# terryye/cuda_FlashAttention

Hardware: AMD Instinct MI355X
Metric: FA2 fwd+bwd TFLOP/s at (B=4,H=16,N=8192,d=128); % MFMA peak (higher is better)
Workload: dtype bf16; 1 GPU; FA2 forward+backward bf16, (B=4,H=16,N=8192,d=128) per GPU, non-causal (BASELINE configs[2]); flops = 14 B H N^2 d; B=4, H=16, N=8192, d=128, parallelism=head-sharded replicas x1

## Files before the change

cuda_flashattention_amd/csrc/fa2_bwd_bf16.hip:

```cpp
#include <type_traits>

#include "fa2_regfile.h"
#include "fa2_launch.h"

namespace fa2 {

constexpr float kNoKeyRC = -1.0e30f;
constexpr float kNoKeyLq = 1.0e30f;

template <int D>
__global__ void __launch_bounds__(256) fa2_bwd_delta_kernel(const __bf16* __restrict__ dO,
                                                            const __bf16* __restrict__ O,
                                                            const float* __restrict__ L,
                                                            float* __restrict__ Dv, float* __restrict__ RC,
                                                            size_t rows, int nq, int q_hs, int q_row0, size_t rc_plane,
                                                            float inv_scale)
{
    const size_t r = ((size_t)blockIdx.x * 256 + threadIdx.x) >> 4;
    const int sub = threadIdx.x & 15;
    const size_t head = r / (size_t)nq, i = r % (size_t)nq;
    const size_t row = head * (size_t)q_hs + i;
    const size_t prow = row + (size_t)q_row0;
    float acc = 0.0f;
    if (r < rows) {
#pragma unroll
        for (int c = sub * 8; c < D; c += 128) {
            const bf16x8 a = *reinterpret_cast<const bf16x8*>(dO + row * D + c);
            const bf16x8 b = *reinterpret_cast<const bf16x8*>(O + row * D + c);
#pragma unroll
            for (int e = 0; e < 8; ++e) acc += (float)a[e] * (float)b[e];
        }
    }
#pragma unroll
    for (int off = 8; off >= 1; off >>= 1) acc += __shfl_xor(acc, off, 16);
    if (r < rows && sub == 0) {
        Dv[prow] = acc;
        const float l = L[row];
        RC[prow] = l == -INFINITY ? kNoKeyRC : -l * inv_scale;
        RC[rc_plane + prow] = -acc;
    }
}

constexpr int kBwdRows = 256;
constexpr int kDqWaves = 4;
constexpr int kDqKV = 64;
constexpr int kDkQ = 32;

typedef __attribute__((address_space(3))) void* lptr_t;

#include "fa2_bwd_dq_body.inc"
// ... 402 lines not shown
            constexpr int RK = A_DK + 16 * (kb * DT + dt) + 4 * g, RV = A_DV + 16 * (kb * DT + dt) + 4 * g;
            bf16x4 a, b;
            a[0] = (__bf16)(aread<RK>() * p.scale); a[1] = (__bf16)(aread<RK + 1>() * p.scale);
            a[2] = (__bf16)(aread<RK + 2>() * p.scale); a[3] = (__bf16)(aread<RK + 3>() * p.scale);
            b[0] = (__bf16)aread<RV>(); b[1] = (__bf16)aread<RV + 1>();
            b[2] = (__bf16)aread<RV + 2>(); b[3] = (__bf16)aread<RV + 3>();
            if (key < N) {
                *reinterpret_cast<bf16x4*>(dKk + 2 * (32 * dt + 8 * g + 4 * h)) = a;
                *reinterpret_cast<bf16x4*>(dVk + 2 * (32 * dt + 8 * g + 4 * h)) = b;
            }
        });
    });
}

template <int D, bool CAUSAL>
__global__ void __launch_bounds__(256, 1) __attribute__((amdgpu_num_vgpr(60))) fa2_bwd_dkdv_kernel(BwdArgs p)
{
    const int ncb = (p.Nk + kDkKeys - 1) / kDkKeys;
    int kvhead, cb;
    map_block(blockIdx.x, p.BH / p.kv_group, ncb, kvhead, cb);
    bwd_dkdv_impl<D, CAUSAL>(p, kvhead, cb);
}

template <int D, bool CAUSAL>
__global__ void __launch_bounds__(256, 1) __attribute__((amdgpu_num_vgpr(60))) fa2_bwd_dkdv_varlen_kernel(VarlenBwdArgs v)
{
    int kvhead, idx;
    map_block(blockIdx.x, v.a.BH / v.a.kv_group, v.n_key_items, kvhead, idx);
    const VarlenItem it = uniform_item(v.key_items, idx);
    bwd_dkdv_impl<D, CAUSAL>(bwd_varlen_view<D>(v.a, it), kvhead, it.block);
}

template <int D, bool CAUSAL>
static hipError_t launch_bwd_one(const BwdArgs& a, hipStream_t stream)
{
    const size_t rows = (size_t)a.BH * a.Nq;
    hipError_t e = hipSuccess;
    if (a.phases & 1) {
        hipLaunchKernelGGL((fa2_bwd_delta_kernel<D>), dim3((unsigned)((rows * 16 + 255) / 256)), dim3(256), 0,
                           stream, (const __bf16*)a.dO, (const __bf16*)a.O, a.L, a.D, a.RC, rows, a.Nq, a.q_hs, a.q_row0,
                           (size_t)a.BH * a.q_hs, 1.0f / a.scale);
        e = hipGetLastError();
        if (e != hipSuccess) return e;
    }
    const int nb = (a.Nq + kBwdRows - 1) / kBwdRows;
    constexpr int lds_dq = 3 * 2 * kDqKV * D * 2;
    constexpr int lds_dk = kDkKeys * D * 2 + 2 * (2 * 2 * kDkQ * D * 2 + 512);
    if (a.phases & 2) {
        e = launch_lds<fa2_bwd_dq_kernel<D, CAUSAL>>(dim3((unsigned)(nb * a.BH)), dim3(256), lds_dq, stream, a);
        if (e != hipSuccess) return e;
    }
    if (a.phases & 4) {
        const int ncb = (a.Nk + kDkKeys - 1) / kDkKeys;
        e = launch_lds<fa2_bwd_dkdv_kernel<D, CAUSAL>>(dim3((unsigned)(ncb * (a.BH / a.kv_group))), dim3(256), lds_dk, stream, a);
    }
    return e;
}

template <int D, bool CAUSAL>
static hipError_t launch_bwd_varlen_one(const VarlenBwdArgs& v, hipStream_t stream)
{
    const BwdArgs& a = v.a;
    const size_t rows = (size_t)a.BH * a.q_hs;
    hipLaunchKernelGGL((fa2_bwd_delta_kernel<D>), dim3((unsigned)((rows * 16 + 255) / 256)), dim3(256), 0, stream,
                       (const __bf16*)a.dO, (const __bf16*)a.O, a.L, a.D, a.RC, rows, a.q_hs, a.q_hs, 0, rows, 1.0f / a.scale);
    hipError_t e = hipGetLastError();
    if (e != hipSuccess) return e;
    constexpr int lds_dq = 3 * 2 * kDqKV * D * 2;
    constexpr int lds_dk = kDkKeys * D * 2 + 2 * (2 * 2 * kDkQ * D * 2 + 512);
    e = launch_lds<fa2_bwd_dq_varlen_kernel<D, CAUSAL>>(dim3((unsigned)(v.n_row_items * a.BH)), dim3(256), lds_dq, stream, v);
    if (e != hipSuccess) return e;
    return launch_lds<fa2_bwd_dkdv_varlen_kernel<D, CAUSAL>>(dim3((unsigned)(v.n_key_items * (a.BH / a.kv_group))), dim3(256), lds_dk,
                                                            stream, v);
}

hipError_t launch_bwd_varlen_bf16(const VarlenBwdArgs& v, hipStream_t stream)
{
    const BwdArgs& a = v.a;
    if (a.kv_group < 1 || a.BH % a.kv_group != 0 || v.n_row_items < 1 || v.n_key_items < 1 || !v.row_items || !v.key_items)
        return hipErrorInvalidValue;
    if (a.d == 128) return a.causal ? launch_bwd_varlen_one<128, true>(v, stream) : launch_bwd_varlen_one<128, false>(v, stream);
    if (a.d == 64) return a.causal ? launch_bwd_varlen_one<64, true>(v, stream) : launch_bwd_varlen_one<64, false>(v, stream);
    return hipErrorInvalidValue;
}

hipError_t launch_bwd_bf16(const BwdArgs& a, hipStream_t stream)
{
    if (a.kv_group < 1 || a.BH % a.kv_group != 0) return hipErrorInvalidValue;
    if (a.d == 128) return a.causal ? launch_bwd_one<128, true>(a, stream) : launch_bwd_one<128, false>(a, stream);
    if (a.d == 64) return a.causal ? launch_bwd_one<64, true>(a, stream) : launch_bwd_one<64, false>(a, stream);
    return hipErrorInvalidValue;
}

}
```

cuda_flashattention_amd/csrc/fa2_bwd_fused.hip:

```cpp
#include <cstdlib>
#include <cstring>
#include <type_traits>

#include "fa2_regfile.h"
#include "fa2_launch.h"

namespace fa2 {

#include "fa2_bwd_fused_body.inc"

typedef __attribute__((address_space(3))) void* fused_lptr_t;

#ifndef FA2_FUSED_DSKEY
#define FA2_FUSED_DSKEY(row) (((row) >> 1) & 7)
#endif

#ifndef FA2_FUSED_DIAG
#define FA2_FUSED_DIAG 0
#endif

constexpr int kFusedRegFile = RF512;

#define FA2_FUSED_CLOBBERS "memory", "vcc", FA2_RF512
#define FA2_FUSED_OPS_128 [r0] "v"(roff[0]), [r1] "v"(roff[1]), [r2] "v"(roff[2]), [r3] "v"(roff[3]), [r4] "v"(roff[4]), [r5] "v"(roff[5]),  \
    [r6] "v"(roff[6]), [r7] "v"(roff[7]), [t0] "v"(toff[0]), [t1] "v"(toff[1]), [t2] "v"(toff[2]), [t3] "v"(toff[3]), [t4] "v"(toff[4]),   \
    [t5] "v"(toff[5]), [t6] "v"(toff[6]), [t7] "v"(toff[7]), [rc] "v"(rcv), [c2] "s"(c2)
#define FA2_FUSED_OPS_64 [r0] "v"(roff[0]), [r1] "v"(roff[1]), [r2] "v"(roff[2]), [r3] "v"(roff[3]), [t0] "v"(toff[0]), [t1] "v"(toff[1]),    \
    [t2] "v"(toff[2]), [t3] "v"(toff[3]), [rc] "v"(rcv), [c2] "s"(c2)

struct FusedStep {
    __amdgpu_buffer_rsrc_t drs, lrs, qrs, grs, rcrs, ctl;
    uint32_t dso, lso, qso, rcso, pvo, mso;
    int need, pval;
};
#define FA2_FUSED_STEP(TEXT, DD, ...)                                                                                                 \
    asm volatile(TEXT                                                                                                                 \
                 : [err] "+s"(err)                                                                                                    \
                 : FA2_FUSED_OPS_##DD, [vm] "i"(VMW), [dqv] "v"(dqv), [drs] "s"(f.drs), [dso] "s"(f.dso), [lrs] "s"(f.lrs), [lso] "s"(f.lso), \
// ... 27 lines not shown

template <int DQT>
__device__ __forceinline__ void fused_dq_atomic(__amdgpu_buffer_rsrc_t rs, uint32_t voff, uint32_t soff)
{
    asm volatile(
        "s_add_u32 s12, %2, 4096\n\ts_add_u32 s13, %2, 8192\n\ts_add_u32 s14, %2, 12288\n\t"
        "buffer_atomic_add_f32 v%c3, %0, %1, %2 offen\n\tbuffer_atomic_add_f32 v%c4, %0, %1, %2 offen offset:512\n\t"
        "buffer_atomic_add_f32 v%c5, %0, %1, %2 offen offset:1024\n\tbuffer_atomic_add_f32 v%c6, %0, %1, %2 offen offset:1536\n\t"
        "buffer_atomic_add_f32 v%c7, %0, %1, s12 offen\n\tbuffer_atomic_add_f32 v%c8, %0, %1, s12 offen offset:512\n\t"
        "buffer_atomic_add_f32 v%c9, %0, %1, s12 offen offset:1024\n\tbuffer_atomic_add_f32 v%c10, %0, %1, s12 offen offset:1536\n\t"
        "buffer_atomic_add_f32 v%c11, %0, %1, s13 offen\n\tbuffer_atomic_add_f32 v%c12, %0, %1, s13 offen offset:512\n\t"
        "buffer_atomic_add_f32 v%c13, %0, %1, s13 offen offset:1024\n\tbuffer_atomic_add_f32 v%c14, %0, %1, s13 offen offset:1536\n\t"
        "buffer_atomic_add_f32 v%c15, %0, %1, s14 offen\n\tbuffer_atomic_add_f32 v%c16, %0, %1, s14 offen offset:512\n\t"
        "buffer_atomic_add_f32 v%c17, %0, %1, s14 offen offset:1024\n\tbuffer_atomic_add_f32 v%c18, %0, %1, s14 offen offset:1536\n\t"
        "s_nop 1"
        : : "v"(voff), "s"(rs), "s"(soff), "i"(DQT), "i"(DQT + 1), "i"(DQT + 2), "i"(DQT + 3), "i"(DQT + 4), "i"(DQT + 5), "i"(DQT + 6),
            "i"(DQT + 7), "i"(DQT + 8), "i"(DQT + 9), "i"(DQT + 10), "i"(DQT + 11), "i"(DQT + 12), "i"(DQT + 13), "i"(DQT + 14),
            "i"(DQT + 15)
        : "memory", "s12", "s13", "s14", "v255");
}

template <int VF, int KS, int S>
__device__ __forceinline__ void fused_load_vfrag(const char* v0, const char* v1)
{
#ifndef FA2_FUSED_KV_NT
#define FA2_FUSED_KV_NT ""
#define FA2_FUSED_KV_AUX 0
#endif
    asm volatile("global_load_dwordx4 v[%c2:%c3], %0, off offset:%c4" FA2_FUSED_KV_NT "\n\tglobal_load_dwordx4 v[%c5:%c6], %1, off offset:%c4" FA2_FUSED_KV_NT
                 : : "v"(v0), "v"(v1), "i"(VF + 4 * S), "i"(VF + 4 * S + 3), "i"(32 * S), "i"(VF + 4 * (KS + S)), "i"(VF + 4 * (KS + S) + 3)
                 : "memory", "v255");
}

template <int DQT>
__device__ __forceinline__ void fused_dq_zero()
{
    static_for<16>([&](auto R) { vset<kFusedRegFile, CL_TOP, DQT + decltype(R)::value>(0u); });
}

constexpr int kCtlTicket = 0, kCtlNextHead = 32 * 16, kCtlError = 32 * 17, kCtlHeadmap = 32 * 18;
constexpr int kHmPad = 16;
constexpr int kSpinLimit = FA2_FUSED_SPIN_LIMIT;

struct FusedArgs {
    BwdArgs b;
    float* dQacc;
    int* ctl;
    int npad;
    const float* rc;
    int fault;
};

#ifdef FA2_TEST_HOOKS
static int g_hook_fault = 0, g_hook_grid = 0, g_hook_last_grid = 0;
extern "C" void fa2_test_set_fused_hooks(int fault, int grid) { g_hook_fault = fault; g_hook_grid = grid; }
extern "C" int fa2_test_last_fused_grid(void) { return g_hook_last_grid; }
#define FA2_HOOK_NOTE_GRID(n) (g_hook_last_grid = (n))
#else
constexpr int g_hook_fault = 0, g_hook_grid = 0;
#define FA2_HOOK_NOTE_GRID(n) ((void)0)
#endif

__device__ __forceinline__ int fused_ctl_ints(int BH, int ncb) { return kCtlHeadmap + 16 * (BH + kHmPad) + 9 * BH * ncb; }

__device__ __forceinline__ int fused_load_sc1(const int* p)
{
    int v;
    asm volatile("global_load_dword %0, %1, off sc1\n\ts_waitcnt vmcnt(0)" : "=v"(v) : "v"(p) : "memory");
    return v;
}
__device__ __forceinline__ void fused_seen_set(int v)
{
    asm volatile("v_mov_b32 v39, %0" : : "s"(v) : "v39");
}

__device__ __forceinline__ int fused_lane_id() { return (int)__builtin_amdgcn_mbcnt_hi(~0u, __builtin_amdgcn_mbcnt_lo(~0u, 0u)); }
template <int OFF>
__device__ __forceinline__ int fused_mail_read(uint32_t lds_addr)
{
    int v;
    asm volatile("v_mov_b32 %0, %1\n\tds_read_b32 %0, %0 offset:%c2\n\ts_waitcnt lgkmcnt(0)" : "=&v"(v) : "s"(lds_addr), "i"(OFF) : "memory");
    return __builtin_amdgcn_readfirstlane(v);
}

__device__ __forceinline__ void fused_store_flag(int* p, int v)
{
    asm volatile("global_store_dword %0, %1, off" : : "v"(p), "v"(v) : "memory");
}

__device__ __forceinline__ bool fused_spin_over(int* ctl, int spins)
{
    if (spins > kSpinLimit) {
        atomicExch(ctl + kCtlError, 1);
        return true;
    }
    return (spins & 1023) == 0 && fused_load_sc1(ctl + kCtlError) != 0;
}

template <bool CHAIN, bool CAUSAL, bool RAGGED = false, bool RECT = false, int HD = 128>
__global__ void __launch_bounds__(256, 1) __attribute__((amdgpu_num_vgpr(39))) fa2_bwd_fused_kernel(FusedArgs fp)
{
    static_assert(CHAIN || !RAGGED, "the atomics form has no ragged variant");
    static_assert(!RECT || (CHAIN && !CAUSAL && !RAGGED), "rectangular blocks: chained, unmasked, aligned");
    static_assert(HD == 128 || (HD == 64 && CHAIN && !RECT), "head_dim 64: chained, square");
    extern __shared__ __attribute__((aligned(16))) char smem[];
    const BwdArgs& p = fp.b;
// ... 37 lines not shown
    for (int dt = 0; dt < DT; ++dt)
#pragma unroll
        for (int jj = 0; jj < 2; ++jj)
            toff[2 * dt + jj] = lbase + QRING + lds_off<D>(8 * jj + 4 * h + trq, 4 * dt + 2 * trcb + (trp >> 1)) + 8 * (trp & 1);
    const uint32_t rcv = lbase + QRING + 2 * TROWS * ROWB + 16 * h;
    static_for<KS>([&](auto S) {
        constexpr int sidx = decltype(S)::value;
        vset<kFusedRegFile, CL_TOP, ROFFK + sidx>(lbase + lds_off<D>(ki + 64 * wave, 2 * sidx + h));
    });
    const int ecol = W ? wave : (wave & 1), ekey0 = W ? 0 : 128 * (wave >> 1);
    static_for<2>([&](auto JJ) {
        constexpr int jj = decltype(JJ)::value;
        vset<kFusedRegFile, CL_TOP, KT + jj>(lbase + ekey0 * ROWB + lds_off<D>(8 * jj + 4 * h + trq, 4 * ecol + 2 * trcb + (trp >> 1)) + 8 * (trp & 1));
        const int row = 8 * jj + 4 * h + trq;
        vset<kFusedRegFile, CL_TOP, DSRD + jj>(lbase + DSB + (ekey0 + row) * 64 + 8 * ((4 * trcb + trp) ^ FA2_FUSED_DSKEY(row)));
    });
    static_for<4>([&](auto C) {
        constexpr int c = decltype(C)::value;
        vset<kFusedRegFile, CL_TOP, DSWR + c>(lbase + DSB + (64 * wave + ki) * 64 + 8 * (((2 * c) | h) ^ FA2_FUSED_DSKEY(ki)));
    });
    const int doff = lds_dma_off<D>(wave * RPI, lane);
    const uint32_t dqv = CHAIN ? (uint32_t)(wave * 4096 + lane * 16) : (uint32_t)(((4 * h) * D + 32 * wave + ki) * 4);
    const auto rc_rsrc = __builtin_amdgcn_make_buffer_rsrc((void*)fp.rc, 0, (int)(2 * rc_plane * 4), 0x00020000);

    int xcc = 0;
    if constexpr (CHAIN) {
        asm volatile("s_getreg_b32 %0, hwreg(HW_REG_XCC_ID, 0, 4)" : "=s"(xcc));
    }
    int* const prog_base = fp.ctl + kCtlHeadmap + 16 * (p.BH + kHmPad);
#ifndef FA2_FUSED_CAUSAL_G
#define FA2_FUSED_CAUSAL_G 2
#endif
    const int G = CAUSAL ? max(1, min(FA2_FUSED_CAUSAL_G, p.BH / 8)) : 1;
    const auto ctl_rsrc = __builtin_amdgcn_make_buffer_rsrc((void*)fp.ctl, 0, CHAIN ? fused_ctl_ints(p.BH, ncb) * 4 : 0, 0x00020000);

    auto take_ticket = [&]() {
        if (wave == 0 && fused_lane_id() == 0) {
            int hd, j = 0;
            do {
                const int u = atomicAdd(fp.ctl + kCtlTicket + 32 * xcc, 1);
                const int r = u % (G * ncb);
                const int k = (u / (G * ncb)) * G + r % G;
                j = r / G;
                hd = -2;
                if (k < p.BH + kHmPad) {
                    int* hm = fp.ctl + kCtlHeadmap + xcc * (p.BH + kHmPad) + k;
                    int v = 0, spins = 0;
                    if (j == 0) {
                        if (k > 0)
                            while ((v = fused_load_sc1(hm - 1)) == 0)
                                if (fused_spin_over(fp.ctl, ++spins)) break;
                        if (k > 0 && v == 0) {
                            v = -1;
                        } else {
                            const int g = atomicAdd(fp.ctl + kCtlNextHead, 1);
                            v = g < p.BH ? g + 1 : -1;
                        }
                        fused_store_flag(hm, v);
                    } else {
                        while ((v = fused_load_sc1(hm)) == 0)
                            if (fused_spin_over(fp.ctl, ++spins)) { v = -1; break; }
                    }
                    hd = v > 0 ? v - 1 : (r % G == 0 ? -2 : -1);
                }
            } while (hd == -1);
            mail[0] = hd;
            mail[1] = j;
            mail[2] = hd >= 0 ? fused_load_sc1(fp.ctl + kCtlError) : 0;
        }
    };
    auto issue_unit_loads = [&](int head_, int cb_) {
        const size_t slab_ = (size_t)(head_ / p.kv_group) * KHS * ROWB;
        const char* Kh_ = (const char*)p.K + slab_;
        const char* Vh_ = (const char*)p.V + slab_;
        const int kw0_ = cb_ * 256 + wave * 64;
        const int lane_u = (int)__builtin_amdgcn_mbcnt_hi(~0u, __builtin_amdgcn_mbcnt_lo(~0u, 0u));
        const int vk0 = RAGGED ? min(kw0_ + (lane_u & 31), N - 1) : kw0_ + (lane_u & 31);
        const int vk1 = RAGGED ? min(kw0_ + 32 + (lane_u & 31), N - 1) : kw0_ + 32 + (lane_u & 31);
        const char* v0 = Vh_ + (size_t)vk0 * ROWB + 16 * (lane_u >> 5);
        const char* v1 = Vh_ + (size_t)vk1 * ROWB + 16 * (lane_u >> 5);
        static_for<KS>([&](auto S) { fused_load_vfrag<VF, KS, decltype(S)::value>(v0, v1); });
        const auto k_rsrc = __builtin_amdgcn_make_buffer_rsrc((void*)Kh_, 0, N * ROWB, 0x00020000);
#pragma unroll
        for (int j = wave; j < 256 / RPI; j += 4)
            __builtin_amdgcn_raw_ptr_buffer_load_lds(k_rsrc, (fused_lptr_t)(smem + j * 1024), 16, doff, (cb_ * 256 + j * RPI) * ROWB, 0, FA2_FUSED_KV_AUX);
    };

    auto next_unit_loads = [&]() {
        if constexpr (CHAIN) {
            take_ticket();
            __syncthreads();
            const int hn = fused_mail_read<0>(mail_addr);
            if (hn >= 0) issue_unit_loads(hn, fused_mail_read<4>(mail_addr));
        }
    };
    next_unit_loads();

    for (;;) {
#ifdef FA2_FUSED_STATS
        const uint64_t s_pull = __builtin_readcyclecounter();
#endif
        int head, cb, err0 = 0;
        if constexpr (CHAIN) {
            head = fused_mail_read<0>(mail_addr);
            cb = fused_mail_read<4>(mail_addr);
            err0 = fused_mail_read<8>(mail_addr);
            if (head < 0) break;
        } else {
            map_block(blockIdx.x, p.BH, ncb, head, cb);
            issue_unit_loads(head, cb);
        }
        const size_t slab = (size_t)head * QHS * ROWB;
        const char* Qh = (const char*)p.Q + slab;
        const char* Gh = (const char*)p.dO + slab;
        const int kw0 = cb * 256 + wave * 64;
        {
            const u32x4 z = {0u, 0u, 0u, 0u};
            static_for<4 * DT>([&](auto T) { azero16<kFusedRegFile, CL_ACC, 16 * decltype(T)::value>(z); });
        }

        const auto q_rsrc = __builtin_amdgcn_make_buffer_rsrc((void*)Qh, 0, NQ * ROWB, 0x00020000);
        const auto g_rsrc = __builtin_amdgcn_make_buffer_rsrc((void*)Gh, 0, NQ * ROWB, 0x00020000);
        const int rcoff = (int)(((wave == 0 ? 0 : rc_plane) + (size_t)head * (RECT ? QHS : NP) + QR0 + (fused_lane_id() & 31)) * 4);
        auto stage = [&](int t, int buf) {
            char* b = smem + QRING + buf * BUFB;
#pragma unroll
            for (int j = wave; j < 2 * NINS; j += 4) {
                const int which = j / NINS, piece = j % NINS;
                const int soff = (t * TROWS + piece * RPI) * ROWB;
                __builtin_amdgcn_raw_ptr_buffer_load_lds(which ? g_rsrc : q_rsrc, (fused_lptr_t)(b + which * (TROWS * ROWB) + piece * 1024),
                                                         16, doff, soff, 0, 0);
            }
            if (wave < 2 && fused_lane_id() < 32)
                __builtin_amdgcn_raw_ptr_buffer_load_lds(rc_rsrc, (fused_lptr_t)(b + 2 * TROWS * ROWB + wave * 128), 4, rcoff, t * TROWS * 4, 0, 0);
        };
        const int n_u = CAUSAL ? ntiles - 8 * cb : ntiles;
        const int niter_u = CAUSAL ? ((n_u + 1 + 5) / 6) * 6 : niter;
        const bool ragged_unit = RAGGED && !CAUSAL && cb == ncb - 1;
        const int first_masked = CAUSAL ? ((n_u - 8) / 6) * 6 : (ragged_unit ? 0 : niter_u);
// ... 91 lines not shown
#endif
                fused_dq_zero<DQT>();
            }
        };
        auto six = [&](auto MASKED, auto FAST_, int t) {
            step(std::integral_constant<int, 0>{}, std::integral_constant<int, 0>{}, MASKED, FAST_, t);
            step(std::integral_constant<int, 1>{}, std::integral_constant<int, 1>{}, MASKED, FAST_, t + 1);
            step(std::integral_constant<int, 2>{}, std::integral_constant<int, 0>{}, MASKED, FAST_, t + 2);
            step(std::integral_constant<int, 0>{}, std::integral_constant<int, 1>{}, MASKED, FAST_, t + 3);
            step(std::integral_constant<int, 1>{}, std::integral_constant<int, 0>{}, MASKED, FAST_, t + 4);
            step(std::integral_constant<int, 2>{}, std::integral_constant<int, 1>{}, MASKED, FAST_, t + 5);
        };
        const int fast_end = CHAIN ? n_u - 2 : -1;
        {
            const int plain_end = first_masked;
            int t = 0;
            asm volatile("" : "+s"(t));
            if (t < plain_end) { six(std::false_type{}, std::false_type{}, t); t += 6; }
#pragma unroll 1
            for (; t + 5 <= fast_end && t < plain_end; t += 6) six(std::false_type{}, std::true_type{}, t);
#pragma unroll 1
            for (; t < plain_end; t += 6) six(std::false_type{}, std::false_type{}, t);
            if constexpr (CHAIN && (CAUSAL || RAGGED)) {
#pragma unroll 1
                for (; t < niter_u; t += 6) six(std::true_type{}, std::false_type{}, t);
            }
        }
        asm volatile("s_waitcnt vmcnt(0) lgkmcnt(0)" ::: "memory");
        if constexpr (CHAIN)
            if (err && !err0 && wave == 0 && fused_lane_id() == 0) atomicExch(fp.ctl + kCtlError, 1);
#ifdef FA2_FUSED_STATS
        const uint64_t s_loop = __builtin_readcyclecounter();
#endif
        next_unit_loads();

        mfma_acc_settle();
        const int lane_ep = (int)__builtin_amdgcn_mbcnt_hi(~0u, __builtin_amdgcn_mbcnt_lo(~0u, 0u));
        const int ki_ep = lane_ep & 31, h_ep = lane_ep >> 5;
        static_for<2>([&](auto KB) {
            constexpr int kb = decltype(KB)::value;
            const int key = kw0 + 32 * kb + ki_ep;
            const size_t slab_k = RECT ? (size_t)head * KHS * ROWB : slab;
            char* const dKb = (char*)p.dK + slab_k;
            char* const dVb = (char*)p.dV + slab_k;
            const uint32_t koff = (uint32_t)key * ROWB + 16u * h_ep;
            char* dKk = dKb + koff;
            char* dVk = dVb + koff;
            static_for<2 * DT>([&](auto G) {
                constexpr int dt = decltype(G)::value / 2, gp = decltype(G)::value % 2;
                constexpr int RK = 16 * (kb * DT + dt) + 8 * gp, RV = 32 * DT + RK;
                auto pack4 = [&](float a, float b, float c, float d, float sc) {
                    bf16x4 v;
                    v[0] = (__bf16)(a * sc); v[1] = (__bf16)(b * sc); v[2] = (__bf16)(c * sc); v[3] = (__bf16)(d * sc);
                    return __builtin_bit_cast(u32x2, v);
                };
                auto emit = [&](u32x2 x, u32x2 y, char* dst) {
                    const auto s0 = __builtin_amdgcn_permlane32_swap(x[0], y[0], false, false);
                    const auto s1 = __builtin_amdgcn_permlane32_swap(x[1], y[1], false, false);
                    const u32x4 o = {s0[0], s1[0], s0[1], s1[1]};
#ifdef FA2_FUSED_ST_NT
                    if (!RAGGED || key < N) __builtin_nontemporal_store(o, reinterpret_cast<u32x4*>(dst + 2 * (32 * dt + 16 * gp)));
#else
                    if (!RAGGED || key < N) *reinterpret_cast<u32x4*>(dst + 2 * (32 * dt + 16 * gp)) = o;
#endif
                };
                emit(pack4(aread<RK>(), aread<RK + 1>(), aread<RK + 2>(), aread<RK + 3>(), p.scale),
                     pack4(aread<RK + 4>(), aread<RK + 5>(), aread<RK + 6>(), aread<RK + 7>(), p.scale), dKk);
                emit(pack4(aread<RV>(), aread<RV + 1>(), aread<RV + 2>(), aread<RV + 3>(), 1.0f),
                     pack4(aread<RV + 4>(), aread<RV + 5>(), aread<RV + 6>(), aread<RV + 7>(), 1.0f), dVk);
            });
        });
#ifdef FA2_FUSED_STATS
        if (CHAIN && wave == 0 && fused_lane_id() == 0) {
            atomicAdd(fp.ctl + kCtlError + 1, st_steps);
            atomicAdd(fp.ctl + kCtlError + 2, st_polls);
            atomicAdd((unsigned long long*)(fp.ctl + kCtlError + 4), (unsigned long long)st_cycles);
            atomicAdd((unsigned long long*)(fp.ctl + kCtlError + 6), (unsigned long long)(__builtin_readcyclecounter() - u0));
            int* rec = prog_base + p.BH * ncb + 8 * (head * ncb + cb);
            rec[0] = xcc; rec[1] = st_cycles; rec[2] = (int)(u0 - s_pull); rec[3] = (int)(__builtin_readcyclecounter() - s_loop);
            *(unsigned long long*)(rec + 4) = u0; *(unsigned long long*)(rec + 6) = __builtin_readcyclecounter();
        }
#endif
        if constexpr (!CHAIN) break;
    }
}

__global__ void __launch_bounds__(256) fa2_bwd_fused_dq_out_kernel(const float* __restrict__ acc, __bf16* __restrict__ dQ, size_t n8, float scale,
                                                                    const int* __restrict__ err)
{
    const float poison = (err && *err) ? __builtin_nanf("") : 0.0f;
    const size_t stride = (size_t)gridDim.x * 256;
    for (size_t i = (size_t)blockIdx.x * 256 + threadIdx.x; i < n8; i += stride) {
        const f32x4 a = reinterpret_cast<const f32x4*>(acc)[2 * i], b = reinterpret_cast<const f32x4*>(acc)[2 * i + 1];
        bf16x8 o;
#pragma unroll
        for (int e = 0; e < 4; ++e) { o[e] = (__bf16)(a[e] * scale + poison); o[4 + e] = (__bf16)(b[e] * scale + poison); }
        reinterpret_cast<bf16x8*>(dQ)[i] = o;
    }
}

__global__ void __launch_bounds__(256) fa2_bwd_fused_dq_out_chain_kernel(const float* __restrict__ acc, __bf16* __restrict__ dQ, size_t n4, float scale,
                                                                          const int* __restrict__ err, int N, int NP, int qhs)
{
    const float poison = *err ? __builtin_nanf("") : 0.0f;
    const size_t stride = (size_t)gridDim.x * 256;
    const size_t tiles = (size_t)(NP / 32);
    for (size_t i = (size_t)blockIdx.x * 256 + threadIdx.x; i < n4; i += stride) {
        const f32x4 a = reinterpret_cast<const f32x4*>(acc)[i];
        const int lane = (int)(i & 63), g = (int)((i >> 6) & 3), wave = (int)((i >> 8) & 3);
        const size_t tg = i >> 10, head = tg / tiles;
        const int row = (int)(tg % tiles) * 32 + 8 * g + 4 * (lane >> 5);
        __bf16* o = dQ + (head * (size_t)qhs + row) * 128 + 32 * wave + (lane & 31);
#pragma unroll
        for (int e = 0; e < 4; ++e)
            if (row + e < N) o[(size_t)e * 128] = (__bf16)(a[e] * scale + poison);
    }
}

__global__ void __launch_bounds__(256) fa2_bwd_fused_dq_out_chain64_kernel(const float* __restrict__ acc, __bf16* __restrict__ dQ, size_t n4h, float scale,
                                                                            const int* __restrict__ err, int N, int NP)
{
    const float poison = *err ? __builtin_nanf("") : 0.0f;
    const size_t stride = (size_t)gridDim.x * 256;
    const size_t tiles = (size_t)(NP / 32);
    for (size_t i = (size_t)blockIdx.x * 256 + threadIdx.x; i < n4h; i += stride) {
        const int lane = (int)(i & 63), g = (int)((i >> 6) & 3), cbk = (int)((i >> 8) & 1);
        const size_t tg = i >> 9, head = tg / tiles;
        const size_t slot = ((tg * 4 + cbk) * 4 + g) * 64 + lane;
        const f32x4 a = reinterpret_cast<const f32x4*>(acc)[slot], b = reinterpret_cast<const f32x4*>(acc)[slot + 2 * 4 * 64];
        const int row = (int)(tg % tiles) * 32 + 8 * g + 4 * (lane >> 5);
        __bf16* o = dQ + (head * (size_t)N + row) * 64 + 32 * cbk + (lane & 31);
#pragma unroll
        for (int e = 0; e < 4; ++e)
            if (row + e < N) o[(size_t)e * 64] = (__bf16)((a[e] + b[e]) * scale + poison);
    }
}

__global__ void __launch_bounds__(256) fa2_bwd_fused_dkdv_out_kernel(const bf16x8* __restrict__ pK, const bf16x8* __restrict__ pV,
                                                                      bf16x8* __restrict__ dK, bf16x8* __restrict__ dV, size_t n8, size_t nkv, int G)
{
    const size_t stride = (size_t)gridDim.x * 256;
    for (size_t i = (size_t)blockIdx.x * 256 + threadIdx.x; i < 2 * nkv * n8; i += stride) {
        const bool isv = i >= nkv * n8;
        const size_t o = isv ? i - nkv * n8 : i, kvh = o / n8, r = o % n8;
        const bf16x8* src = (isv ? pV : pK) + kvh * (size_t)G * n8 + r;
        float s[8] = {};
        for (int g = 0; g < G; ++g) {
            const bf16x8 x = src[(size_t)g * n8];
#pragma unroll
// ... 41 lines not shown

hipError_t bwd_fused_clear_error(int* ctl, hipStream_t stream)
{
    return launch_fill_f32(reinterpret_cast<float*>(ctl + kCtlError), 1, 0.0f, stream);
}

size_t bwd_fused_kvpart_bytes(int BH, int N, int d) { return (size_t)2 * BH * N * d * 2; }
size_t bwd_fused_ctl_bytes(int BH, int N) { return (size_t)(kCtlHeadmap + 16 * (BH + kHmPad) + 9 * BH * ((N + 255) / 256)) * sizeof(int); }

template <int HD>
static hipError_t launch_chained_square(bool causal, bool ragged, dim3 grid, int lds, hipStream_t stream, const FusedArgs& fa)
{
    if (causal)
        return ragged ? launch_lds<fa2_bwd_fused_kernel<true, true, true, false, HD>>(grid, dim3(256), lds, stream, fa)
                      : launch_lds<fa2_bwd_fused_kernel<true, true, false, false, HD>>(grid, dim3(256), lds, stream, fa);
    return ragged ? launch_lds<fa2_bwd_fused_kernel<true, false, true, false, HD>>(grid, dim3(256), lds, stream, fa)
                  : launch_lds<fa2_bwd_fused_kernel<true, false, false, false, HD>>(grid, dim3(256), lds, stream, fa);
}

hipError_t launch_bwd_fused_bf16(const BwdArgs& a, float* dQacc, int* ctl, int mode, hipStream_t stream, float* rcpad, void* kvpart)
{
    const int npad = (a.Nk + 255) / 256 * 256;
    const bool ragged = npad != a.Nk;
    const bool rect = a.Nq != a.Nk || a.q_hs != a.Nq || a.k_hs != a.Nk || a.q_row0 != 0;
    if ((a.d != 128 && a.d != 64) || a.Nk < 1 || a.Nq < 1) return hipErrorInvalidValue;
    if (a.d == 64 && (mode != 1 || rect)) return hipErrorInvalidValue;
    if (rect && (mode != 1 || a.causal || ragged || a.Nq % 32 != 0 || a.q_row0 < 0 || a.q_hs < a.q_row0 + a.Nq || a.k_hs < a.Nk))
        return hipErrorInvalidValue;
    if (ragged && (mode != 1 || !rcpad)) return hipErrorInvalidValue;
    const bool grouped = a.kv_group > 1;
    if (a.kv_group < 1 || a.BH % a.kv_group != 0 || (grouped && (mode != 1 || rect || !kvpart))) return hipErrorInvalidValue;
    if (a.causal && (mode != 1 || a.causal_shift != 0)) return hipErrorInvalidValue;
    hipError_t e = hipSuccess;
    if (a.phases & 1) {
        BwdArgs d = a;
        d.phases = 1;
        e = launch_bwd_bf16(d, stream);
        if (e != hipSuccess) return e;
    }
    if (!(a.phases & 8)) return hipSuccess;
    const size_t elems = (size_t)a.BH * (rect ? a.Nq : npad) * 128;
    const int units = a.BH * (npad / 256);
    if (ragged) {
        const size_t n = (size_t)2 * a.BH * npad;
        hipLaunchKernelGGL(fa2_bwd_fused_rcpad_kernel, dim3((unsigned)((n + 255) / 256)), dim3(256), 0, stream, (const float*)a.RC, rcpad,
                           a.BH, a.Nk, npad);
        e = hipGetLastError();
        if (e != hipSuccess) return e;
    }
    FusedArgs fa{a, dQacc, ctl, npad, ragged ? (const float*)rcpad : (const float*)a.RC, g_hook_fault};
    const size_t part_elems = (size_t)a.BH * a.Nk * a.d;
    if (grouped) {
        fa.b.dK = kvpart;
        fa.b.dV = (__bf16*)kvpart + part_elems;
    }
    const int lds = (a.d == 64 ? FA2_FUSED64_LDS : FA2_FUSED_LDS) + 16;
    if (mode == 0) {
        e = launch_fill_f32(dQacc, elems, 0.0f, stream);
        if (e != hipSuccess) return e;
        e = bwd_fused_clear_error(ctl, stream);
        if (e != hipSuccess) return e;
        e = launch_lds<fa2_bwd_fused_kernel<false, false>>(dim3((unsigned)units), dim3(256), lds, stream, fa);
    } else {
        static int cus[64] = {};
        int dev = 0;
        e = hipGetDevice(&dev);
        if (e != hipSuccess) return e;
        if (dev < 0 || dev >= 64) return hipErrorInvalidDevice;
        if (!cus[dev]) {
            e = hipDeviceGetAttribute(&cus[dev], hipDeviceAttributeMultiprocessorCount, dev);
            if (e != hipSuccess) return e;
        }
        e = launch_fill_f32(reinterpret_cast<float*>(ctl), bwd_fused_ctl_bytes(a.BH, a.Nk) / sizeof(float), 0.0f, stream);
        if (e != hipSuccess) return e;
        int avail = cus[dev] - (a.reserve_cus > 0 ? a.reserve_cus : 0);
        if (avail < 1) avail = 1;
        int wgs = units < avail ? units : avail;
        if (g_hook_grid >= 1 && g_hook_grid < wgs) wgs = g_hook_grid;
        FA2_HOOK_NOTE_GRID(wgs);
        const dim3 grid((unsigned)wgs);
        if (rect)
            e = launch_lds<fa2_bwd_fused_kernel<true, false, false, true>>(grid, dim3(256), lds, stream, fa);
        else
            e = a.d == 64 ? launch_chained_square<64>(a.causal, ragged, grid, lds, stream, fa)
                          : launch_chained_square<128>(a.causal, ragged, grid, lds, stream, fa);
    }
    if (e != hipSuccess) return e;
    if (mode == 0)
        hipLaunchKernelGGL(fa2_bwd_fused_dq_out_kernel, dim3(2048), dim3(256), 0, stream, dQacc, (__bf16*)a.dQ, elems / 8, a.scale,
                           (const int*)nullptr);
    else if (a.d == 64)
        hipLaunchKernelGGL(fa2_bwd_fused_dq_out_chain64_kernel, dim3(4096), dim3(256), 0, stream, dQacc, (__bf16*)a.dQ, elems / 8, a.scale,
                           ctl + kCtlError, a.Nk, npad);
    else
        hipLaunchKernelGGL(fa2_bwd_fused_dq_out_chain_kernel, dim3(4096), dim3(256), 0, stream, dQacc, (__bf16*)a.dQ, elems / 4, a.scale,
                           ctl + kCtlError, rect ? a.Nq : a.Nk, rect ? a.Nq : npad, rect ? a.q_hs : a.Nk);
    e = hipGetLastError();
    if (e != hipSuccess || !grouped) return e;
    hipLaunchKernelGGL(fa2_bwd_fused_dkdv_out_kernel, dim3(4096), dim3(256), 0, stream, (const bf16x8*)fa.b.dK, (const bf16x8*)fa.b.dV,
                       (bf16x8*)a.dK, (bf16x8*)a.dV, (size_t)a.Nk * a.d / 8, (size_t)(a.BH / a.kv_group), a.kv_group);
    return hipGetLastError();
}

}
```

cuda_flashattention_amd/csrc/fa2_launch.h:

```cpp
#pragma once
#include <hip/hip_runtime.h>
#include <stddef.h>

namespace fa2 {

struct FwdArgs {
    const void* Q;
    const void* K;
    const void* V;
    void* O;
    float* L;
    float* Oacc;
    float* M;
    int BH, Nq, Nk, d;
    float scale;
    int causal;
    int causal_shift;
    int resume;
    int finalize;
    int q_hs, k_hs;
    int kv_group;
};

hipError_t launch_fwd1_bf16(const FwdArgs& a, hipStream_t stream);
// ... 8 lines not shown
hipError_t launch_accumulate_bf16(float* acc, const void* src, size_t rows, size_t cols, size_t pitch, int init, hipStream_t stream);
hipError_t launch_finalize_state(const float* Oacc, const float* M, float* L, void* O, size_t rows, int d, hipStream_t stream);

struct FwdFp8Args {
    const void* Q; const void* K; const void* V;
    void* Vt;
    float* kn;
    void* O;
    float* L;
    int BH, N, Npad, d;
    float scale;
    int causal;
    float o_scale;
};
hipError_t launch_fwd_fp8(const FwdFp8Args& a, hipStream_t stream);

struct BwdArgs {
    const void* Q; const void* K; const void* V; const void* O; const void* dO;
    const float* L;
    void* dQ; void* dK; void* dV;
    float* D;
    float* RC;
    int BH, Nq, Nk, d;
    int q_hs, k_hs;
    int q_row0;
    float scale;
    int causal;
    int causal_shift;
    int phases;
    int reserve_cus;
    int kv_group;
};

hipError_t launch_bwd_bf16(const BwdArgs& a, hipStream_t stream);
struct VarlenBwdArgs {
    BwdArgs a;
    const VarlenItem* row_items; const VarlenItem* key_items;
    int n_row_items, n_key_items;
};
hipError_t launch_bwd_varlen_bf16(const VarlenBwdArgs& v, hipStream_t stream);
size_t bwd_fused_ctl_bytes(int BH, int N);
size_t bwd_fused_kvpart_bytes(int BH, int N, int d);
hipError_t launch_bwd_fused_bf16(const BwdArgs& a, float* dQacc, int* ctl, int mode, hipStream_t stream, float* rcpad = nullptr,
                                 void* kvpart = nullptr);
bool bwd_fused_device_ok(const char** why);
hipError_t bwd_fused_read_error(const int* ctl, int* err, hipStream_t stream);
hipError_t bwd_fused_clear_error(int* ctl, hipStream_t stream);

struct F32Args {
    const float* Q; const float* K; const float* V; float* O; float* L;
    const float* dO; float* dQ; float* dK; float* dV; float* D;
    int BH, N, d;
    float scale;
    int causal;
    int phases;
    int Nk;
    float* M;
    int resume, finalize;
};
hipError_t launch_fwd_f32(const F32Args& a, hipStream_t stream);
hipError_t launch_bwd_f32(const F32Args& a, hipStream_t stream);

template <auto K, typename A>
inline hipError_t launch_lds(dim3 grid, dim3 block, int lds, hipStream_t stream, const A& arg)
{
    static bool done[64] = {};
    int dev = 0;
// ... 23 lines not shown
```

Baseline: 1319 TFLOP/s.

## Convert dQ accumulator to bf16 inside persistent fused backward kernel

```diff
diff --git a/cuda_flashattention_amd/csrc/fa2_bwd_bf16.hip b/cuda_flashattention_amd/csrc/fa2_bwd_bf16.hip
--- a/cuda_flashattention_amd/csrc/fa2_bwd_bf16.hip
+++ b/cuda_flashattention_amd/csrc/fa2_bwd_bf16.hip
@@ -14,8 +14,9 @@
                                                             const float* __restrict__ L,
                                                             float* __restrict__ Dv, float* __restrict__ RC,
                                                             size_t rows, int nq, int q_hs, int q_row0, size_t rc_plane,
-                                                            float inv_scale)
-{
+                                                            float inv_scale, int* __restrict__ zero, size_t nzero)
+{
+    for (size_t z = (size_t)blockIdx.x * 256 + threadIdx.x; z < nzero; z += (size_t)gridDim.x * 256) zero[z] = 0;
     const size_t r = ((size_t)blockIdx.x * 256 + threadIdx.x) >> 4;
     const int sub = threadIdx.x & 15;
     const size_t head = r / (size_t)nq, i = r % (size_t)nq;
@@ -484,14 +485,14 @@
 }
 
 template <int D, bool CAUSAL>
-static hipError_t launch_bwd_one(const BwdArgs& a, hipStream_t stream)
+static hipError_t launch_bwd_one(const BwdArgs& a, hipStream_t stream, int* zero, size_t nzero)
 {
     const size_t rows = (size_t)a.BH * a.Nq;
     hipError_t e = hipSuccess;
     if (a.phases & 1) {
         hipLaunchKernelGGL((fa2_bwd_delta_kernel<D>), dim3((unsigned)((rows * 16 + 255) / 256)), dim3(256), 0,
                            stream, (const __bf16*)a.dO, (const __bf16*)a.O, a.L, a.D, a.RC, rows, a.Nq, a.q_hs, a.q_row0,
-                           (size_t)a.BH * a.q_hs, 1.0f / a.scale);
+                           (size_t)a.BH * a.q_hs, 1.0f / a.scale, zero, nzero);
         e = hipGetLastError();
         if (e != hipSuccess) return e;
     }
@@ -515,7 +516,8 @@
     const BwdArgs& a = v.a;
     const size_t rows = (size_t)a.BH * a.q_hs;
     hipLaunchKernelGGL((fa2_bwd_delta_kernel<D>), dim3((unsigned)((rows * 16 + 255) / 256)), dim3(256), 0, stream,
-                       (const __bf16*)a.dO, (const __bf16*)a.O, a.L, a.D, a.RC, rows, a.q_hs, a.q_hs, 0, rows, 1.0f / a.scale);
+                       (const __bf16*)a.dO, (const __bf16*)a.O, a.L, a.D, a.RC, rows, a.q_hs, a.q_hs, 0, rows, 1.0f / a.scale,
+                       (int*)nullptr, (size_t)0);
     hipError_t e = hipGetLastError();
     if (e != hipSuccess) return e;
     constexpr int lds_dq = 3 * 2 * kDqKV * D * 2;
@@ -536,11 +538,11 @@
     return hipErrorInvalidValue;
 }
 
-hipError_t launch_bwd_bf16(const BwdArgs& a, hipStream_t stream)
-{
-    if (a.kv_group < 1 || a.BH % a.kv_group != 0) return hipErrorInvalidValue;
-    if (a.d == 128) return a.causal ? launch_bwd_one<128, true>(a, stream) : launch_bwd_one<128, false>(a, stream);
-    if (a.d == 64) return a.causal ? launch_bwd_one<64, true>(a, stream) : launch_bwd_one<64, false>(a, stream);
+hipError_t launch_bwd_bf16(const BwdArgs& a, hipStream_t stream, int* zero, size_t nzero)
+{
+    if (a.kv_group < 1 || a.BH % a.kv_group != 0 || (nzero && !(a.phases & 1))) return hipErrorInvalidValue;
+    if (a.d == 128) return a.causal ? launch_bwd_one<128, true>(a, stream, zero, nzero) : launch_bwd_one<128, false>(a, stream, zero, nzero);
+    if (a.d == 64) return a.causal ? launch_bwd_one<64, true>(a, stream, zero, nzero) : launch_bwd_one<64, false>(a, stream, zero, nzero);
     return hipErrorInvalidValue;
 }
 
diff --git a/cuda_flashattention_amd/csrc/fa2_bwd_fused.hip b/cuda_flashattention_amd/csrc/fa2_bwd_fused.hip
--- a/cuda_flashattention_amd/csrc/fa2_bwd_fused.hip
+++ b/cuda_flashattention_amd/csrc/fa2_bwd_fused.hip
@@ -4,6 +4,7 @@
 
 #include "fa2_regfile.h"
 #include "fa2_launch.h"
+#include "fa2_fused_tickets.h"
 
 namespace fa2 {
 
@@ -97,6 +98,34 @@
                  : "memory", "v255");
 }
 
+struct FusedDqSlot { int row, col; };
+__host__ __device__ constexpr FusedDqSlot fused_dq_slot(int tile, int wave, int g, int lane)
+{
+    return FusedDqSlot{32 * tile + 8 * g + 4 * (lane >> 5), 32 * wave + (lane & 31)};
+}
+__device__ __forceinline__ __bf16 fused_dq_round(float a, float scale, float poison) { return (__bf16)(a * scale + poison); }
+
+template <int R0>
+__device__ __forceinline__ void fused_conv_load_tile(__amdgpu_buffer_rsrc_t rs, uint32_t voff, uint32_t soff)
+{
+    asm volatile("buffer_load_dwordx4 v[%c3:%c4], %0, %1, %2 offen sc1\n\tbuffer_load_dwordx4 v[%c5:%c6], %0, %1, %2 offen offset:1024 sc1\n\t"
+                 "buffer_load_dwordx4 v[%c7:%c8], %0, %1, %2 offen offset:2048 sc1\n\tbuffer_load_dwordx4 v[%c9:%c10], %0, %1, %2 offen offset:3072 sc1"
+                 : : "v"(voff), "s"(rs), "s"(soff), "i"(R0), "i"(R0 + 3), "i"(R0 + 4), "i"(R0 + 7), "i"(R0 + 8), "i"(R0 + 11), "i"(R0 + 12),
+                     "i"(R0 + 15)
+                 : "memory", "v255");
+}
+
+template <int R>
+__device__ __forceinline__ void fused_conv_store_slot(__bf16* o, float scale)
+{
+    asm volatile("v_fma_f32 v%c2, v%c2, %1, 0\n\tv_fma_f32 v%c3, v%c3, %1, 0\n\tv_fma_f32 v%c4, v%c4, %1, 0\n\tv_fma_f32 v%c5, v%c5, %1, 0\n\t"
+                 "v_cvt_pk_bf16_f32 v%c2, v%c2, v%c3\n\tv_cvt_pk_bf16_f32 v%c4, v%c4, v%c5\n\t"
+                 "global_store_short %0, v%c2, off\n\tglobal_store_short_d16_hi %0, v%c2, off offset:256\n\t"
+                 "global_store_short %0, v%c4, off offset:512\n\tglobal_store_short_d16_hi %0, v%c4, off offset:768"
+                 : : "v"(o), "s"(scale), "i"(R), "i"(R + 1), "i"(R + 2), "i"(R + 3)
+                 : "memory", "v255");
+}
+
 template <int DQT>
 __device__ __forceinline__ void fused_dq_zero()
 {
@@ -114,15 +143,17 @@
     int npad;
     const float* rc;
     int fault;
+    int inline_dq;
 };
 
 #ifdef FA2_TEST_HOOKS
-static int g_hook_fault = 0, g_hook_grid = 0, g_hook_last_grid = 0;
+static int g_hook_fault = 0, g_hook_grid = 0, g_hook_last_grid = 0, g_hook_dq_pass = 0;
 extern "C" void fa2_test_set_fused_hooks(int fault, int grid) { g_hook_fault = fault; g_hook_grid = grid; }
+extern "C" void fa2_test_force_fused_dq_pass(int on) { g_hook_dq_pass = on; }
 extern "C" int fa2_test_last_fused_grid(void) { return g_hook_last_grid; }
 #define FA2_HOOK_NOTE_GRID(n) (g_hook_last_grid = (n))
 #else
-constexpr int g_hook_fault = 0, g_hook_grid = 0;
+constexpr int g_hook_fault = 0, g_hook_grid = 0, g_hook_dq_pass = 0;
 #define FA2_HOOK_NOTE_GRID(n) ((void)0)
 #endif
 
@@ -134,9 +165,25 @@
     asm volatile("global_load_dword %0, %1, off sc1\n\ts_waitcnt vmcnt(0)" : "=v"(v) : "v"(p) : "memory");
     return v;
 }
+__device__ __forceinline__ void fused_load2_sc1(const int* p, const int* q, int& a, int& b)
+{
+    asm volatile("global_load_dword %0, %2, off sc1\n\tglobal_load_dword %1, %3, off sc1\n\ts_waitcnt vmcnt(0)"
+                 : "=&v"(a), "=&v"(b) : "v"(p), "v"(q) : "memory");
+}
 __device__ __forceinline__ void fused_seen_set(int v)
 {
     asm volatile("v_mov_b32 v39, %0" : : "s"(v) : "v39");
+}
+
+__device__ __forceinline__ void fused_seen_prefetch(const int* p)
+{
+    asm volatile("global_load_dword v39, %0, off sc1" : : "v"(p) : "memory", "v39");
+}
+__device__ __forceinline__ int fused_seen_get()
+{
+    int v;
+    asm volatile("s_waitcnt vmcnt(0)\n\tv_mov_b32 %0, v39" : "=v"(v) : : "memory");
+    return v;
 }
 
 __device__ __forceinline__ int fused_lane_id() { return (int)__builtin_amdgcn_mbcnt_hi(~0u, __builtin_amdgcn_mbcnt_lo(~0u, 0u)); }
@@ -240,25 +287,36 @@
 #define FA2_FUSED_CAUSAL_G 2
 #endif
     const int G = CAUSAL ? max(1, min(FA2_FUSED_CAUSAL_G, p.BH / 8)) : 1;
+    constexpr bool CONV = CHAIN && !CAUSAL && !RAGGED && !RECT && HD == 128;
+    constexpr int CVR = VF + 8 * KS;
+    static_assert(!CONV || CVR + 128 <= DQT + 16, "a share's 128 registers: the tile and fragment slots and the dQ tile, nothing else");
+    const bool conv_on = CONV && fp.inline_dq != 0;
     const auto ctl_rsrc = __builtin_amdgcn_make_buffer_rsrc((void*)fp.ctl, 0, CHAIN ? fused_ctl_ints(p.BH, ncb) * 4 : 0, 0x00020000);
 
-    auto take_ticket = [&]() {
+    auto take_ticket = [&](int spec) {
         if (wave == 0 && fused_lane_id() == 0) {
-            int hd, j = 0;
+            int hd, j = 0, cv = -1;
+            bool fetched = false;
+            if constexpr (CONV)
+                if (conv_on && spec >= 0) {
+                    fused_seen_prefetch(prog_base + spec * ncb + ncb - 1);
+                    fetched = true;
+                }
             do {
                 const int u = atomicAdd(fp.ctl + kCtlTicket + 32 * xcc, 1);
-                const int r = u % (G * ncb);
-                const int k = (u / (G * ncb)) * G + r % G;
-                j = r / G;
+                const FusedTicket t = fused_ticket_decode(u, ncb, G);
+                const int k = t.chain;
+                j = t.block;
                 hd = -2;
-                if (k < p.BH + kHmPad) {
+                cv = -1;
+                if (!fused_chain_past_map(k, p.BH, kHmPad)) {
                     int* hm = fp.ctl + kCtlHeadmap + xcc * (p.BH + kHmPad) + k;
-                    int v = 0, spins = 0;
+                    int v = 0, vp = -1, spins = 0;
                     if (j == 0) {
                         if (k > 0)
-                            while ((v = fused_load_sc1(hm - 1)) == 0)
+                            while ((vp = fused_load_sc1(hm - 1)) == 0)
                                 if (fused_spin_over(fp.ctl, ++spins)) break;
-                        if (k > 0 && v == 0) {
+                        if (k > 0 && vp == 0) {
                             v = -1;
                         } else {
                             const int g = atomicAdd(fp.ctl + kCtlNextHead, 1);
@@ -266,15 +324,34 @@
                         }
                         fused_store_flag(hm, v);
                     } else {
-                        while ((v = fused_load_sc1(hm)) == 0)
-                            if (fused_spin_over(fp.ctl, ++spins)) { v = -1; break; }
+                        const bool both = CONV && conv_on && k > 0;
+                        for (;;) {
+                            if (both) fused_load2_sc1(hm, hm - 1, v, vp);
+                            else v = fused_load_sc1(hm);
+                            if (v != 0 && (!both || vp != 0)) break;
+                            if (fused_spin_over(fp.ctl, ++spins)) { v = -1; vp = -1; break; }
+                        }
                     }
-                    hd = v > 0 ? v - 1 : (r % G == 0 ? -2 : -1);
+                    const FusedUnit un = fused_unit(v, CONV ? vp : -1, t.member, conv_on);
+                    hd = un.kind == kFusedCompute ? un.head : un.kind == kFusedConvert ? -3 : un.kind == kFusedSkip ? -1 : -2;
+                    if constexpr (CONV) cv = un.conv_head;
+                    if constexpr (CONV) if (cv >= 0) {
+                        const int* pw = prog_base + cv * ncb + ncb - 1;
+                        const int need = fused_share_need(j, fused_share_tiles(ntiles, ncb));
+                        int seen = fetched && cv == spec ? fused_seen_get() : 0;
+                        spins = 0;
+                        while (seen < need) {
+                            if (fused_spin_over(fp.ctl, ++spins)) { cv = -1; break; }
+                            seen = fused_load_sc1(pw);
+                        }
+                        if (cv < 0 && hd == -3) hd = -2;
+                    }
                 }
             } while (hd == -1);
             mail[0] = hd;
             mail[1] = j;
             mail[2] = hd >= 0 ? fused_load_sc1(fp.ctl + kCtlError) : 0;
+            if constexpr (CONV) mail[3] = cv;
         }
     };
     auto issue_unit_loads = [&](int head_, int cb_) {
@@ -294,15 +371,42 @@
             __builtin_amdgcn_raw_ptr_buffer_load_lds(k_rsrc, (fused_lptr_t)(smem + j * 1024), 16, doff, (cb_ * 256 + j * RPI) * ROWB, 0, FA2_FUSED_KV_AUX);
     };
 
-    auto next_unit_loads = [&]() {
+    int cv_head = -1, cv_share = 0;
+    auto next_unit_loads = [&](int spec) {
         if constexpr (CHAIN) {
-            take_ticket();
+            take_ticket(spec);
             __syncthreads();
             const int hn = fused_mail_read<0>(mail_addr);
+            if constexpr (CONV) {
+                cv_head = fused_mail_read<12>(mail_addr);
+                cv_share = fused_mail_read<4>(mail_addr);
+                if (cv_head >= 0) {
+                    const auto cv_rsrc = __builtin_amdgcn_make_buffer_rsrc((void*)(fp.dQacc + (size_t)cv_head * NPQ * DQW), 0, NPQ * DQW * 4, 0x00020000);
+                    static_for<8>([&](auto T) {
+                        constexpr int tt = decltype(T)::value;
+                        fused_conv_load_tile<CVR + 16 * tt>(cv_rsrc, dqv, (uint32_t)((cv_share * 8 + tt) * TROWS * DQW * 4));
+                    });
+                }
+            }
             if (hn >= 0) issue_unit_loads(hn, fused_mail_read<4>(mail_addr));
         }
     };
-    next_unit_loads();
+    auto finish_convert = [&]() {
+        if constexpr (CONV) {
+            if (cv_head >= 0) {
+                asm volatile("s_waitcnt vmcnt(0)" ::: "memory");
+                const int lane_c = (int)__builtin_amdgcn_mbcnt_hi(~0u, __builtin_amdgcn_mbcnt_lo(~0u, 0u));
+                const FusedDqSlot s0 = fused_dq_slot(cv_share * 8, wave, 0, lane_c);
+                __bf16* const o0 = (__bf16*)p.dQ + ((size_t)cv_head * N + s0.row) * D + s0.col;
+                static_for<32>([&](auto I) {
+                    constexpr int tt = decltype(I)::value / 4, g = decltype(I)::value % 4, R = CVR + 4 * decltype(I)::value;
+                    fused_conv_store_slot<R>(o0 + fused_dq_slot(tt, 0, g, 0).row * D, p.scale);
+                });
+            }
+        }
+    };
+    next_unit_loads(-1);
+    finish_convert();
 
     for (;;) {
 #ifdef FA2_FUSED_STATS
@@ -313,6 +417,14 @@
             head = fused_mail_read<0>(mail_addr);
             cb = fused_mail_read<4>(mail_addr);
             err0 = fused_mail_read<8>(mail_addr);
+            if constexpr (CONV) {
+                if (head == -3) {
+                    __syncthreads();
+                    next_unit_loads(cv_head);
+                    finish_convert();
+                    continue;
+                }
+            }
             if (head < 0) break;
         } else {
             map_block(blockIdx.x, p.BH, ncb, head, cb);
@@ -470,7 +582,7 @@
 #ifdef FA2_FUSED_STATS
         const uint64_t s_loop = __builtin_readcyclecounter();
 #endif
-        next_unit_loads();
+        next_unit_loads(head);
 
         mfma_acc_settle();
         const int lane_ep = (int)__builtin_amdgcn_mbcnt_hi(~0u, __builtin_amdgcn_mbcnt_lo(~0u, 0u));
@@ -519,6 +631,7 @@
             *(unsigned long long*)(rec + 4) = u0; *(unsigned long long*)(rec + 6) = __builtin_readcyclecounter();
         }
 #endif
+        finish_convert();
         if constexpr (!CHAIN) break;
     }
 }
@@ -547,12 +660,20 @@
         const f32x4 a = reinterpret_cast<const f32x4*>(acc)[i];
         const int lane = (int)(i & 63), g = (int)((i >> 6) & 3), wave = (int)((i >> 8) & 3);
         const size_t tg = i >> 10, head = tg / tiles;
-        const int row = (int)(tg % tiles) * 32 + 8 * g + 4 * (lane >> 5);
-        __bf16* o = dQ + (head * (size_t)qhs + row) * 128 + 32 * wave + (lane & 31);
+        const FusedDqSlot sl = fused_dq_slot((int)(tg % tiles), wave, g, lane);
+        const int row = sl.row;
+        __bf16* o = dQ + (head * (size_t)qhs + row) * 128 + sl.col;
 #pragma unroll
         for (int e = 0; e < 4; ++e)
-            if (row + e < N) o[(size_t)e * 128] = (__bf16)(a[e] * scale + poison);
-    }
+            if (row + e < N) o[(size_t)e * 128] = fused_dq_round(a[e], scale, poison);
+    }
+}
+
+__global__ void __launch_bounds__(256) fa2_bwd_fused_dq_poison_kernel(u32x4* __restrict__ dQ, size_t n8, const int* __restrict__ err)
+{
+    if (*err == 0) return;
+    const u32x4 nan8 = {0x7fc07fc0u, 0x7fc07fc0u, 0x7fc07fc0u, 0x7fc07fc0u};
+    for (size_t i = (size_t)blockIdx.x * 256 + threadIdx.x; i < n8; i += (size_t)gridDim.x * 256) dQ[i] = nan8;
 }
 
 __global__ void __launch_bounds__(256) fa2_bwd_fused_dq_out_chain64_kernel(const float* __restrict__ acc, __bf16* __restrict__ dQ, size_t n4h, float scale,
@@ -660,10 +781,11 @@
     if (a.kv_group < 1 || a.BH % a.kv_group != 0 || (grouped && (mode != 1 || rect || !kvpart))) return hipErrorInvalidValue;
     if (a.causal && (mode != 1 || a.causal_shift != 0)) return hipErrorInvalidValue;
     hipError_t e = hipSuccess;
+    const bool fold_fill = mode == 1 && (a.phases & 1) && (a.phases & 8);
     if (a.phases & 1) {
         BwdArgs d = a;
         d.phases = 1;
-        e = launch_bwd_bf16(d, stream);
+        e = launch_bwd_bf16(d, stream, fold_fill ? ctl : nullptr, fold_fill ? bwd_fused_ctl_bytes(a.BH, a.Nk) / sizeof(int) : 0);
         if (e != hipSuccess) return e;
     }
     if (!(a.phases & 8)) return hipSuccess;
@@ -676,7 +798,8 @@
         e = hipGetLastError();
         if (e != hipSuccess) return e;
     }
-    FusedArgs fa{a, dQacc, ctl, npad, ragged ? (const float*)rcpad : (const float*)a.RC, g_hook_fault};
+    const bool inline_dq = mode == 1 && !rect && !ragged && !a.causal && a.d == 128 && !g_hook_dq_pass;
+    FusedArgs fa{a, dQacc, ctl, npad, ragged ? (const float*)rcpad : (const float*)a.RC, g_hook_fault, inline_dq ? 1 : 0};
     const size_t part_elems = (size_t)a.BH * a.Nk * a.d;
     if (grouped) {
         fa.b.dK = kvpart;
@@ -699,7 +822,7 @@
             e = hipDeviceGetAttribute(&cus[dev], hipDeviceAttributeMultiprocessorCount, dev);
             if (e != hipSuccess) return e;
         }
-        e = launch_fill_f32(reinterpret_cast<float*>(ctl), bwd_fused_ctl_bytes(a.BH, a.Nk) / sizeof(float), 0.0f, stream);
+        if (!fold_fill) e = launch_fill_f32(reinterpret_cast<float*>(ctl), bwd_fused_ctl_bytes(a.BH, a.Nk) / sizeof(float), 0.0f, stream);
         if (e != hipSuccess) return e;
         int avail = cus[dev] - (a.reserve_cus > 0 ? a.reserve_cus : 0);
         if (avail < 1) avail = 1;
@@ -717,6 +840,8 @@
     if (mode == 0)
         hipLaunchKernelGGL(fa2_bwd_fused_dq_out_kernel, dim3(2048), dim3(256), 0, stream, dQacc, (__bf16*)a.dQ, elems / 8, a.scale,
                            (const int*)nullptr);
+    else if (inline_dq)
+        hipLaunchKernelGGL(fa2_bwd_fused_dq_poison_kernel, dim3(256), dim3(256), 0, stream, (u32x4*)a.dQ, elems / 8, (const int*)(ctl + kCtlError));
     else if (a.d == 64)
         hipLaunchKernelGGL(fa2_bwd_fused_dq_out_chain64_kernel, dim3(4096), dim3(256), 0, stream, dQacc, (__bf16*)a.dQ, elems / 8, a.scale,
                            ctl + kCtlError, a.Nk, npad);
diff --git a/cuda_flashattention_amd/csrc/fa2_fused_tickets.h b/cuda_flashattention_amd/csrc/fa2_fused_tickets.h
--- /dev/null
+++ b/cuda_flashattention_amd/csrc/fa2_fused_tickets.h
@@ -0,0 +1,45 @@
+#pragma once
+
+namespace fa2 {
+
+enum FusedUnitKind {
+    kFusedCompute = 0,
+    kFusedConvert = 1,
+    kFusedSkip = 2,
+    kFusedEnd = 3
+};
+
+struct FusedTicket {
+    int chain;
+    int block;
+    int member;
+};
+
+constexpr FusedTicket fused_ticket_decode(int u, int ncb, int G)
+{
+    const int r = u % (G * ncb);
+    return FusedTicket{(u / (G * ncb)) * G + r % G, r / G, r % G};
+}
+
+struct FusedUnit {
+    int kind;
+    int head;
+    int conv_head;
+};
+
+constexpr FusedUnit fused_unit(int hm, int hm_prev, int member, bool convert)
+{
+    const int conv = convert && hm_prev > 0 ? hm_prev - 1 : -1;
+    if (hm > 0) return FusedUnit{kFusedCompute, hm - 1, conv};
+    if (conv >= 0) return FusedUnit{kFusedConvert, -1, conv};
+    return FusedUnit{member == 0 ? kFusedEnd : kFusedSkip, -1, -1};
+}
+
+constexpr bool fused_chain_past_map(int chain, int BH, int pad) { return chain >= BH + pad; }
+
+constexpr int fused_share_tiles(int ntiles, int ncb) { return ntiles / ncb; }
+constexpr int fused_share_need(int j, int share_tiles) { return (j + 1) * share_tiles; }
+constexpr int fused_share_waits_for(int chain, int ncb) { return (chain - 1) * ncb + ncb - 1; }
+constexpr int fused_ticket_of(int chain, int block, int ncb) { return chain * ncb + block; }
+
+}
diff --git a/cuda_flashattention_amd/csrc/fa2_launch.h b/cuda_flashattention_amd/csrc/fa2_launch.h
--- a/cuda_flashattention_amd/csrc/fa2_launch.h
+++ b/cuda_flashattention_amd/csrc/fa2_launch.h
@@ -64,7 +64,7 @@
     int kv_group;
 };
 
-hipError_t launch_bwd_bf16(const BwdArgs& a, hipStream_t stream);
+hipError_t launch_bwd_bf16(const BwdArgs& a, hipStream_t stream, int* zero = nullptr, size_t nzero = 0);
 struct VarlenBwdArgs {
     BwdArgs a;
     const VarlenItem* row_items; const VarlenItem* key_items;
```

After: 1330 TFLOP/s, median of 6. No clear change (+0.8%).
